# skhu101/SHERF

Measured on AMD Instinct MI355X. Metric: rendered rays/sec at 512x512x64 samples (ImportanceRenderer.forward), higher is better.
Workload: dtype f16 MFMA (fp16 operands rounded to nearest, one product, fp32 accumulate), fp32 elsewhere

## Files before the change

sherf_amd/csrc/mlp.hip:

```cpp
#include "common.h"

#include <algorithm>

namespace {

typedef __bf16 bf16x8 __attribute__((ext_vector_type(8)));
typedef __bf16 bf16x2 __attribute__((ext_vector_type(2)));
typedef _Float16 f16x8 __attribute__((ext_vector_type(8)));
typedef _Float16 f16x2 __attribute__((ext_vector_type(2)));
typedef float f32x16 __attribute__((ext_vector_type(16)));
typedef uint32_t u32x4 __attribute__((ext_vector_type(4)));

constexpr int N_CHUNKS = 49;
constexpr int N_STEPS = 43;
constexpr int NW = 4;
constexpr int NSLOT = 3;
constexpr int BIAS_LN = N_CHUNKS;

__host__ __device__ constexpr int step_units(int s) {
    return s < 4 ? 10 : s < 20 ? 8 : s < 26 ? ((s - 20) % 3 == 0 ? 10 : 8) : s < 42 ? 8 : 4;
}
__host__ __device__ constexpr int step_unit(int s, int u) {
    int c = -1, kb = 0;
    if (s == 0) { if (u < 2) { c = 0; kb = u; } else { c = 1 + (u - 2) / 2; kb = (u - 2) % 2; } }
// ... 294 lines not shown
        AFrag<PREC> nxt;
        const bool pre = i + 1 < NB || MORE;
        if (pre) nxt = load_units<PREC>(s + (u0 + 2 * (i + 1)) * UNIT);
        const BFrag<PREC>& b0 = b[PAIR ? i : 2 * i];
        const BFrag<PREC>& b1 = b[PAIR ? i : 2 * i + 1];
        if constexpr (PREC == 1) mfma_block<PREC>(acc0, acc1, cur.h0, cur.l0, cur.h1, cur.l1, b0.hi, b0.lo, b1.hi, b1.lo);
        else mfma_block<PREC>(acc0, acc1, cur.h0, cur.h0, cur.h1, cur.h1, b0.hi, b0.hi, b1.hi, b1.hi);
        if (pre) cur = nxt;
    }
}
template <int PREC, int NK, bool MORE = false>
__device__ __forceinline__ void mma_pair(const char* s, int u0, const BFrag<PREC>* b, f32x16& acc0, f32x16& acc1, AFrag<PREC>& cur) {
    mma_chains<PREC, NK, true, MORE>(s, u0, b, acc0, acc1, cur);
}
template <int PREC, int NK>
__device__ __forceinline__ void mma_splitk(const char* s, int u0, const BFrag<PREC>* b, f32x16& acc0, f32x16& acc1, AFrag<PREC>& cur) {
    static_assert(NK % 2 == 0, "even / odd K-block chains");
    mma_chains<PREC, NK / 2, false, false>(s, u0, b, acc0, acc1, cur);
}

#ifndef SHERF_MLP_PERMLANE
#define SHERF_MLP_PERMLANE 1
#endif
__device__ __forceinline__ float xhalf_sum(float v) {
#if SHERF_MLP_PERMLANE
    const uint32_t b = __builtin_bit_cast(uint32_t, v);
    const auto r = __builtin_amdgcn_permlane32_swap(b, b, false, false);
    return __builtin_bit_cast(float, (uint32_t)r[0]) + __builtin_bit_cast(float, (uint32_t)r[1]);
#else
    return v + __shfl_xor(v, 32);
#endif
}

template <int PREC, class C>
__device__ __forceinline__ void layer_norm(const C& cx, const f32x16& x, int ln_idx, BFrag<PREC>& k0, BFrag<PREC>& k1) {
    const f32x16 g = bias_tile(cx, BIAS_LN + 2 * ln_idx), bt = bias_tile(cx, BIAS_LN + 2 * ln_idx + 1);
    f32x16 y;
    if constexpr (PREC == 1) {
        float s = 0.f;
#pragma unroll
        for (int r = 0; r < 16; ++r) s += x[r];
        s = xhalf_sum(s);
        const float mean = s * (1.0f / 32.0f);
        float q = 0.f;
#pragma unroll
        for (int r = 0; r < 16; ++r) { float d = x[r] - mean; q += d * d; }
        q = xhalf_sum(q);
        const float inv = rsqrt_(q * (1.0f / 32.0f) + 1e-5f);
#pragma unroll
        for (int r = 0; r < 16; ++r) y[r] = (x[r] - mean) * inv * g[r] + bt[r];
    } else {
        float s = 0.f, q = 0.f;
#pragma unroll
        for (int r = 0; r < 16; ++r) { s += x[r]; q = __builtin_fmaf(x[r], x[r], q); }
        s = xhalf_sum(s); q = xhalf_sum(q);
        const float mean = s * (1.0f / 32.0f), ex2 = q * (1.0f / 32.0f);
        float var = fmaxf(__builtin_fmaf(-mean, mean, ex2), 0.0f);
        if (__ballot(ex2 > 257.0f * var) != 0) {
            float q2 = 0.f;
#pragma unroll
            for (int r = 0; r < 16; ++r) { const float d = x[r] - mean; q2 = __builtin_fmaf(d, d, q2); }
            var = xhalf_sum(q2) * (1.0f / 32.0f);
        }
        const float inv = rsqrt_(var + 1e-5f), off = -mean * inv;
#pragma unroll
        for (int r = 0; r < 16; ++r) y[r] = __builtin_fmaf(__builtin_fmaf(x[r], inv, off), g[r], bt[r]);
    }
    split_tile<PREC>(y, k0, k1);
}

__device__ __forceinline__ void sincos_exact_phase(float a, float* s, float* c) { sherf_sincos_exact_phase(a, s, c); }

template <int PREC, int NF, int NKB>
__device__ __forceinline__ void pe_frags(int h, float x, float y, float z, BFrag<PREC> (&out)[NKB]) {
    if constexpr ((SHERF_MLP_ABLATE & 512) != 0) {
#pragma unroll
        for (int kb = 0; kb < NKB; ++kb) out[kb] = make_frag<PREC>(x, y, z, 0.f, 0.f, 0.f, 0.f, 0.f);
        return;
    }
    float f[NKB * 16];
#pragma unroll
    for (int i = 0; i < NKB * 16; ++i) f[i] = 0.f;
    f[0] = x; f[1] = y; f[2] = z;
    const float v3[3] = {x, y, z};
#pragma unroll
    for (int q = 0; q < NF; ++q) {
#pragma unroll
        for (int a = 0; a < 3; ++a) {
            float s, c;
            sincos_exact_phase(v3[a] * (float)(1 << q), &s, &c);
            if (3 + 6 * q + a < NKB * 16) f[3 + 6 * q + a] = s;
            if (6 + 6 * q + a < NKB * 16) f[6 + 6 * q + a] = c;
        }
    }
#pragma unroll
    for (int kb = 0; kb < NKB; ++kb) {
        float v[8];
#pragma unroll
        for (int e = 0; e < 8; ++e) v[e] = h ? f[16 * kb + 8 + e] : f[16 * kb + e];
        out[kb] = make_frag<PREC>(v[0], v[1], v[2], v[3], v[4], v[5], v[6], v[7]);
    }
}

#ifndef SHERF_MLP_PK_RELU
#define SHERF_MLP_PK_RELU 1
#endif
__device__ __forceinline__ uint32_t relu2_f16(uint32_t p) {
    f16x2 v = __builtin_bit_cast(f16x2, p);
    v = __builtin_elementwise_max(v, f16x2{(_Float16)0.0f, (_Float16)0.0f});
    return __builtin_bit_cast(uint32_t, v);
}

template <int PREC, bool RELU>
__device__ __forceinline__ void finish_pair(f32x16& acc0, f32x16& acc1, BFrag<PREC>* out) {
    mfma_settle(acc0, acc1);
    if constexpr ((SHERF_MLP_ABLATE & 1024) != 0) {
#pragma unroll
        for (int f = 0; f < 4; ++f)
#pragma unroll
            for (int e = 0; e < 4; ++e) out[f].hi[e] = __builtin_bit_cast(uint32_t, f < 2 ? acc0[4 * f + e] : acc1[4 * (f - 2) + e]);
        __builtin_amdgcn_sched_barrier(0);
        return;
    }
    constexpr bool PK = RELU && PREC == 2 && SHERF_MLP_PK_RELU;
    if constexpr (RELU && !PK) {
// ... 23 lines not shown
template <int PREC, bool RING, bool PRE = false, bool PEM = false>
__device__ __forceinline__ void transformer_tile(Ctx<PREC>& cx, const float4* __restrict__ tokens, const float* __restrict__ extras, int64_t tile,
                                                 BFrag<PREC> (&z0b)[2], BFrag<PREC> (&z1b)[2], f32x16 (&tok)[3], const u32x4* __restrict__ pef = nullptr) {
    const int j = cx.lane & 31, h = cx.h;
    if (cx.notrans) {
        if constexpr (!PRE) load_tokens(tokens, tile, j, h, tok);
        split_tile<PREC>(tok[0], z0b[0], z0b[1]);
        split_tile<PREC>(tok[1], z1b[0], z1b[1]);
        if constexpr (RING) { advance(cx, 0); advance(cx, 1); }
        __builtin_amdgcn_sched_barrier(0);
        return;
    }
    {
        if constexpr (!PRE) load_tokens(tokens, tile, j, h, tok);
        const float* ex = extras + tile * 12 * 32 + j;
        if constexpr ((SHERF_MLP_ABLATE & 256) != 0) {
            split_tile<PREC>(tok[0] + tok[2], z0b[0], z0b[1]);
            split_tile<PREC>(tok[1] + tok[2], z1b[0], z1b[1]);
            if constexpr (RING) { advance(cx, 0); advance(cx, 1); }
            return;
        }

        const char* s = RING ? cx.slot(0) : cx.lds;
        {
            BFrag<PREC> b[1][2];
            if constexpr (PEM) { b[0][0].hi = pef[(tile * 7 + 5) * 64 + cx.lane]; b[0][1].hi = pef[(tile * 7 + 6) * 64 + cx.lane]; }
            else pe_frags<PREC, 5, 2>(h, ex[192], ex[224], ex[256], b[0]);
            f32x16 acc[1] = {bias_tile(cx, 0)};
            mma_cols<PREC, 2, 1>(s, 0, b, acc);
            tok[2] += acc[0];
        }
        BFrag<PREC> ln[3][2];
#pragma unroll
        for (int t = 0; t < 3; ++t) layer_norm<PREC>(cx, tok[t], 0, ln[t][0], ln[t][1]);
        float qa[2][16], qb[2][8];
        {
            BFrag<PREC> b2[2][2] = {{ln[0][0], ln[0][1]}, {ln[1][0], ln[1][1]}};
            f32x16 acc[2] = {bias_tile(cx, 1), bias_tile(cx, 1)};
            mma_cols<PREC, 2, 2>(s, 2, b2, acc);
#pragma unroll
            for (int i = 0; i < 2; ++i)
#pragma unroll
                for (int r = 0; r < 16; ++r) qa[i][r] = acc[i][r];
            f32x16 acc2[2] = {bias_tile(cx, 2), bias_tile(cx, 2)};
            mma_cols<PREC, 2, 2>(s, 4, b2, acc2);
#pragma unroll
            for (int i = 0; i < 2; ++i)
#pragma unroll
                for (int r = 0; r < 8; ++r) qb[i][r] = acc2[i][r];
        }
        float dot[2][3][3];
        float o[2][3][8];
        float v0[3][8];
#pragma unroll
        for (int t = 0; t < 3; ++t) {
            const BFrag<PREC> (&lt)[1][2] = reinterpret_cast<const BFrag<PREC> (&)[1][2]>(ln[t]);
            f32x16 acc[1] = {bias_tile(cx, 3)};
            mma_cols<PREC, 2, 1>(s, 6, lt, acc);
#pragma unroll
            for (int i = 0; i < 2; ++i) {
                float d0 = 0.f, d1 = 0.f;
#pragma unroll
                for (int r = 0; r < 8; ++r) { d0 += qa[i][r] * acc[0][r]; d1 += qa[i][8 + r] * acc[0][8 + r]; }
                dot[i][0][t] = d0; dot[i][1][t] = d1;
            }
        }
#pragma unroll
        for (int t = 0; t < 3; ++t) {
            const BFrag<PREC> (&lt)[1][2] = reinterpret_cast<const BFrag<PREC> (&)[1][2]>(ln[t]);
            f32x16 acc[1] = {bias_tile(cx, 4)};
            mma_cols<PREC, 2, 1>(s, 8, lt, acc);
#pragma unroll
            for (int i = 0; i < 2; ++i) {
                float d2 = 0.f;
#pragma unroll
                for (int r = 0; r < 8; ++r) d2 += qb[i][r] * acc[0][r];
                dot[i][2][t] = d2;
            }
#pragma unroll
            for (int r = 0; r < 8; ++r) v0[t][r] = acc[0][8 + r];
        }
        if constexpr (RING) advance(cx, 0);
#pragma unroll
        for (int i = 0; i < 2; ++i)
#pragma unroll
            for (int hd = 0; hd < 3; ++hd) {
                float d[3];
#pragma unroll
                for (int t = 0; t < 3; ++t) d[t] = xhalf_sum(dot[i][hd][t]) * 0.25f;
                float m = fmaxf(d[0], fmaxf(d[1], d[2]));
                float e0 = exp_(d[0] - m), e1 = exp_(d[1] - m), e2 = exp_(d[2] - m);
                float inv = rcp_(e0 + e1 + e2);
                dot[i][hd][0] = e0 * inv; dot[i][hd][1] = e1 * inv; dot[i][hd][2] = e2 * inv;
            }
#pragma unroll
        for (int i = 0; i < 2; ++i)
#pragma unroll
            for (int r = 0; r < 8; ++r) o[i][0][r] = dot[i][0][0] * v0[0][r] + dot[i][0][1] * v0[1][r] + dot[i][0][2] * v0[2][r];
        s = RING ? cx.slot(1) : cx.lds + step_pieces<PREC>(0) * 1024;
#pragma unroll
        for (int i = 0; i < 2; ++i)
#pragma unroll
            for (int r = 0; r < 8; ++r) { o[i][1][r] = 0.f; o[i][2][r] = 0.f; }
#pragma unroll
        for (int t = 0; t < 3; ++t) {
            const BFrag<PREC> (&lt)[1][2] = reinterpret_cast<const BFrag<PREC> (&)[1][2]>(ln[t]);
            f32x16 acc[1] = {bias_tile(cx, 5)};
            mma_cols<PREC, 2, 1>(s, 0, lt, acc);
#pragma unroll
            for (int i = 0; i < 2; ++i)
#pragma unroll
                for (int r = 0; r < 8; ++r) {
                    o[i][1][r] += dot[i][1][t] * acc[0][r];
                    o[i][2][r] += dot[i][2][t] * acc[0][8 + r];
                }
        }
        f32x16 y[2];
        {
            BFrag<PREC> ob[2][3];
#pragma unroll
            for (int i = 0; i < 2; ++i)
#pragma unroll
// ... 31 lines not shown
#pragma unroll
                for (int r = 0; r < 16; ++r) acc[i][r] = gelu_<PREC != 1>(acc[i][r]);
                split_tile<PREC>(acc[i], gb[i][0], gb[i][1]);
            }
            f32x16 acc2[2] = {bias_tile(cx, 8), bias_tile(cx, 8)};
            mma_cols<PREC, 2, 2>(s, 7, gb, acc2);
            if constexpr (RING) advance(cx, 1);
            f32x16 za = acc2[0] + y[0], zb = acc2[1] + y[1];
            split_tile<PREC>(za, z0b[0], z0b[1]);
            split_tile<PREC>(zb, z1b[0], z1b[1]);
        }
    }
    __builtin_amdgcn_sched_barrier(0);
}

template <int PREC>
__device__ __forceinline__ void decoder_tile(Ctx<PREC>& cx, const int32_t* __restrict__ counters, const BFrag<PREC> (&z0b)[2], const BFrag<PREC> (&z1b)[2],
                                             const float (&xc)[3], const float (&vc)[3], int64_t tile, bool live, int64_t nv, float4* __restrict__ out) {
    const int j = cx.lane & 31, h = cx.h;
    if constexpr (SHERF_MLP_DECODER_PRIO > 0) __builtin_amdgcn_s_setprio(SHERF_MLP_DECODER_PRIO);
    int step = 2;
    BFrag<PREC> ha[8], hb[8];
    AFrag<PREC> cur = load_units<PREC>(cx.slot(step));
#define SHERF_NEXT_STEP() do { step_wait(cx, step); cur = load_units<PREC>(cx.slot(step + 1)); dma_issue(cx, step + NSLOT); ++step; } while (0)
#define SHERF_LAYER128(C0, IN, OUT, RELU)                                                             \
    _Pragma("unroll") for (int P = 0; P < 2; ++P) {                                                   \
        f32x16 acc0 = bias_tile(cx, (C0) + 2 * P), acc1 = bias_tile(cx, (C0) + 2 * P + 1);            \
        mma_pair<PREC, 4>(cx.slot(step), 0, IN, acc0, acc1, cur);                                     \
        SHERF_NEXT_STEP();                                                                            \
        mma_pair<PREC, 4>(cx.slot(step), 0, IN + 4, acc0, acc1, cur);                                 \
        SHERF_NEXT_STEP();                                                                            \
        finish_pair<PREC, RELU>(acc0, acc1, OUT + 4 * P);                                             \
    }
    {
        BFrag<PREC> pe[3];
        pe_frags<PREC, 6, 3>(h, xc[0], xc[1], xc[2], pe);
#pragma unroll
        for (int P = 0; P < 2; ++P) {
            f32x16 acc0 = bias_tile(cx, 9 + 2 * P), acc1 = bias_tile(cx, 10 + 2 * P);
            const char* s = cx.slot(step);
            mma_pair<PREC, 3, true>(s, 0, pe, acc0, acc1, cur);
            mma_pair<PREC, 2>(s, 6, z0b, acc0, acc1, cur);
            SHERF_NEXT_STEP();
            finish_pair<PREC, true>(acc0, acc1, ha + 4 * P);
        }
    }
    SHERF_LAYER128(13, ha, hb, true)
    SHERF_LAYER128(17, hb, ha, true)
    SHERF_LAYER128(21, ha, hb, true)
    SHERF_LAYER128(25, hb, ha, true)
    {
        float x0 = xc[0], x1 = xc[1], x2 = xc[2];
        asm volatile("" : "+v"(x0), "+v"(x1), "+v"(x2));
        BFrag<PREC> pe[3];
        pe_frags<PREC, 6, 3>(h, x0, x1, x2, pe);
#pragma unroll
        for (int P = 0; P < 2; ++P) {
            f32x16 acc0 = bias_tile(cx, 29 + 2 * P), acc1 = bias_tile(cx, 30 + 2 * P);
            const char* s = cx.slot(step);
            mma_pair<PREC, 3, true>(s, 0, pe, acc0, acc1, cur);
            mma_pair<PREC, 2>(s, 6, z0b, acc0, acc1, cur);
            SHERF_NEXT_STEP();
            mma_pair<PREC, 4>(cx.slot(step), 0, ha, acc0, acc1, cur);
            SHERF_NEXT_STEP();
            mma_pair<PREC, 4>(cx.slot(step), 0, ha + 4, acc0, acc1, cur);
            SHERF_NEXT_STEP();
            finish_pair<PREC, true>(acc0, acc1, hb + 4 * P);
        }
    }
    SHERF_LAYER128(33, hb, ha, true)
    SHERF_LAYER128(37, ha, hb, true)
    SHERF_LAYER128(41, hb, ha, false)
    float sigma;
    {
        f32x16 acc0 = bias_tile(cx, 45), acc1 = {0.f, 0.f, 0.f, 0.f, 0.f, 0.f, 0.f, 0.f, 0.f, 0.f, 0.f, 0.f, 0.f, 0.f, 0.f, 0.f};
        mma_splitk<PREC, 8>(cx.slot(step), 0, hb, acc0, acc1, cur);
        SHERF_NEXT_STEP();
        mfma_settle(acc0, acc1);
        sigma = acc0[0] + acc1[0];
        __builtin_amdgcn_sched_barrier(0);
    }
    BFrag<PREC> gb[4];
    {
        BFrag<PREC> pv[2];
        pe_frags<PREC, 4, 2>(h, vc[0], vc[1], vc[2], pv);
        f32x16 acc0 = bias_tile(cx, 46), acc1 = bias_tile(cx, 47);
        mma_pair<PREC, 4>(cx.slot(step), 0, ha, acc0, acc1, cur);
        SHERF_NEXT_STEP();
// ... 53 lines not shown
        __builtin_amdgcn_sched_barrier(0);
        fill(f0 + i);
        __builtin_amdgcn_sched_barrier(0);
        if (pre) cur = nxt;
    }
}

template <int PREC, bool PEM = false>
__device__ __forceinline__ void decoder_tile_p(Ctx<PREC>& cx, const int32_t* __restrict__ counters, const BFrag<PREC> (&z0b)[2], const BFrag<PREC> (&z1b)[2],
                                               const float (&xc)[3], const float (&vc)[3], int64_t tile, bool live, int64_t nv, float4* __restrict__ out,
                                               const u32x4* __restrict__ pef = nullptr) {
    const int j = cx.lane & 31, h = cx.h;
    if constexpr (SHERF_MLP_DECODER_PRIO > 0) __builtin_amdgcn_s_setprio(SHERF_MLP_DECODER_PRIO);
    int step = 2;
    BFrag<PREC> ha[8], hb[8];
    if constexpr ((SHERF_MLP_ABLATE & 2048) != 0) {
#pragma unroll
        for (int i = 0; i < 8; ++i) { ha[i] = z0b[i & 1]; hb[i] = z1b[i & 1]; }
    }
    f32x16 X0, X1, Y0, Y1;
    AFrag<PREC> cur = load_units<PREC>(cx.slot(step));
    const f32x16 zero = {0.f, 0.f, 0.f, 0.f, 0.f, 0.f, 0.f, 0.f, 0.f, 0.f, 0.f, 0.f, 0.f, 0.f, 0.f, 0.f};
    auto none = [](int) {};
#define SHERF_NEXT_STEP() do { step_wait(cx, step); cur = load_units<PREC>(cx.slot(step + 1)); dma_issue(cx, step + NSLOT); ++step; } while (0)
#define SHERF_LAYER128_P(C0, IN, OUT, RELU, PREV_RELU, NX0, NX1)                                                                              \
    mma_chains_f<PREC, 4, true, false>(cx.slot(step), 0, IN, X0, X1, cur, 0, [&](int i) { epi_piece<PREC, PREV_RELU>(Y0, Y1, IN + 4, i); }); \
    SHERF_NEXT_STEP();                                                                                                                         \
    mma_chains_f<PREC, 4, true, false>(cx.slot(step), 0, IN + 4, X0, X1, cur, 0, [&](int i) { if (i == 0) { Y0 = bias_tile(cx, (C0) + 2); Y1 = bias_tile(cx, (C0) + 3); } }); \
    SHERF_NEXT_STEP();                                                                                                                         \
    mma_chains_f<PREC, 4, true, false>(cx.slot(step), 0, IN, Y0, Y1, cur, 0, [&](int i) { epi_piece<PREC, RELU>(X0, X1, OUT, i); });           \
    SHERF_NEXT_STEP();                                                                                                                         \
    mma_chains_f<PREC, 4, true, false>(cx.slot(step), 0, IN + 4, Y0, Y1, cur, 0, [&](int i) { if (i == 0) { X0 = bias_tile(cx, NX0); X1 = (NX1) < 0 ? zero : bias_tile(cx, (NX1) < 0 ? 0 : (NX1)); } }); \
    SHERF_NEXT_STEP();
    {
        BFrag<PREC> pe[3];
        if constexpr (PEM) {
#pragma unroll
            for (int kb = 0; kb < 3; ++kb) pe[kb].hi = pef[(tile * 7 + kb) * 64];
        } else pe_frags<PREC, 6, 3>(h, xc[0], xc[1], xc[2], pe);
        X0 = bias_tile(cx, 9); X1 = bias_tile(cx, 10);
        const char* s = cx.slot(step);
        mma_chains_f<PREC, 3, true, true>(s, 0, pe, X0, X1, cur, 0, [&](int i) { if (i == 0) { Y0 = bias_tile(cx, 11); Y1 = bias_tile(cx, 12); } });
        mma_chains_f<PREC, 2, true, false>(s, 6, z0b, X0, X1, cur, 3, none);
        SHERF_NEXT_STEP();
        s = cx.slot(step);
        auto carry = [&](int i) { if (i < 4) epi_piece<PREC, true>(X0, X1, ha, i); else { X0 = bias_tile(cx, 13); X1 = bias_tile(cx, 14); } };
        mma_chains_f<PREC, 3, true, true>(s, 0, pe, Y0, Y1, cur, 0, carry);
        mma_chains_f<PREC, 2, true, false>(s, 6, z0b, Y0, Y1, cur, 3, carry);
        SHERF_NEXT_STEP();
    }
    SHERF_LAYER128_P(13, ha, hb, true, true, 17, 18)
    SHERF_LAYER128_P(17, hb, ha, true, true, 21, 22)
    SHERF_LAYER128_P(21, ha, hb, true, true, 25, 26)
    SHERF_LAYER128_P(25, hb, ha, true, true, 29, 30)
    {
        float x0 = xc[0], x1 = xc[1], x2 = xc[2];
        asm volatile("" : "+v"(x0), "+v"(x1), "+v"(x2));
        BFrag<PREC> pe[3];
        if constexpr (PEM) {
            const u32x4* pp = pef;
            asm volatile("" : "+v"(pp));
#pragma unroll
            for (int kb = 0; kb < 3; ++kb) pe[kb].hi = pp[(tile * 7 + kb) * 64];
        } else pe_frags<PREC, 6, 3>(h, x0, x1, x2, pe);
        const char* s = cx.slot(step);
        auto carry0 = [&](int i) { if (i < 4) epi_piece<PREC, true>(Y0, Y1, ha + 4, i); };
        mma_chains_f<PREC, 3, true, true>(s, 0, pe, X0, X1, cur, 0, carry0);
        mma_chains_f<PREC, 2, true, false>(s, 6, z0b, X0, X1, cur, 3, carry0);
        SHERF_NEXT_STEP();
        mma_chains_f<PREC, 4, true, false>(cx.slot(step), 0, ha, X0, X1, cur, 0, [&](int i) { if (i == 0) { Y0 = bias_tile(cx, 31); Y1 = bias_tile(cx, 32); } });
        SHERF_NEXT_STEP();
        mma_chains_f<PREC, 4, true, false>(cx.slot(step), 0, ha + 4, X0, X1, cur, 0, none);
        SHERF_NEXT_STEP();
        s = cx.slot(step);
        auto carry1 = [&](int i) { if (i < 4) epi_piece<PREC, true>(X0, X1, hb, i); };
        mma_chains_f<PREC, 3, true, true>(s, 0, pe, Y0, Y1, cur, 0, carry1);
        mma_chains_f<PREC, 2, true, false>(s, 6, z0b, Y0, Y1, cur, 3, carry1);
        SHERF_NEXT_STEP();
        mma_chains_f<PREC, 4, true, false>(cx.slot(step), 0, ha, Y0, Y1, cur, 0, [&](int i) { if (i == 0) { X0 = bias_tile(cx, 33); X1 = bias_tile(cx, 34); } });
        SHERF_NEXT_STEP();
        mma_chains_f<PREC, 4, true, false>(cx.slot(step), 0, ha + 4, Y0, Y1, cur, 0, none);
        SHERF_NEXT_STEP();
    }
    SHERF_LAYER128_P(33, hb, ha, true, true, 37, 38)
    SHERF_LAYER128_P(37, ha, hb, true, true, 41, 42)
    SHERF_LAYER128_P(41, hb, ha, false, true, 45, -1)
    float sigma;
    BFrag<PREC> gb[4];
    {
        mma_chains_f<PREC, 4, false, false>(cx.slot(step), 0, hb, X0, X1, cur, 0, [&](int i) {
            epi_piece<PREC, false>(Y0, Y1, ha + 4, i);
            if (i == 3) { Y0 = bias_tile(cx, 46); Y1 = bias_tile(cx, 47); }
        });
        SHERF_NEXT_STEP();
        BFrag<PREC> pv[2];
        if constexpr (PEM) { pv[0].hi = pef[(tile * 7 + 3) * 64]; pv[1].hi = pef[(tile * 7 + 4) * 64]; }
        else pe_frags<PREC, 4, 2>(h, vc[0], vc[1], vc[2], pv);
// ... 467 lines not shown
            z1b[kb].hi = zp[(4 + 2 * kb) * 64]; z1b[kb].lo = zp[(4 + 2 * kb + 1) * 64];
        } else {
            z0b[kb].hi = zp[kb * 64]; z1b[kb].hi = zp[(2 + kb) * 64];
        }
    }
    float xc[3], vc[3];
    const float* ex = extras + tile * 12 * 32 + (cx.lane & 31);
    xc[0] = ex[0]; xc[1] = ex[32]; xc[2] = ex[64]; vc[0] = ex[96]; vc[1] = ex[128]; vc[2] = ex[160];
    decoder_tile<PREC>(cx, counters, z0b, z1b, xc, vc, tile, live, nv, out);
    SHERF_TRACE_FLUSH(cx);
}

}

#if SHERF_MLP_TRACE
extern "C" int sherf_mlp_set_trace(void* buf, int every) {
    SHERF_HIP_CHECK(hipMemcpyToSymbol(HIP_SYMBOL(g_mlp_trace), &buf, sizeof(buf)));
    SHERF_HIP_CHECK(hipMemcpyToSymbol(HIP_SYMBOL(g_mlp_trace_every), &every, sizeof(every)));
    return SHERF_OK;
}
#endif

extern "C" int sherf_mlp_stream_layout(int prec, int32_t* n_steps, int32_t* step_pieces_host, int32_t* units, int32_t max_steps) {
    SHERF_CHECK_ARG(prec >= 0 && prec <= 2 && n_steps && step_pieces_host && units && max_steps >= N_STEPS);
    *n_steps = N_STEPS;
    for (int s = 0; s < N_STEPS; ++s) {
        step_pieces_host[s] = prec == 1 ? step_pieces<1>(s) : step_pieces<0>(s);
        for (int u = 0; u < 10; ++u) units[s * 10 + u] = u < step_units(s) ? step_unit(s, u) : -1;
    }
    return SHERF_OK;
}

namespace {
__global__ void __launch_bounds__(256) mlp_pack_stream_kernel(const float* __restrict__ flat, const int32_t* __restrict__ src, int64_t n16, int prec,
                                                              uint16_t* __restrict__ out, const int32_t* __restrict__ bias_src, int n_bias,
                                                              float* __restrict__ bias_out, int32_t* __restrict__ flag) {
    const int64_t i = (int64_t)blockIdx.x * 256 + threadIdx.x;
    int bad = 0;
    if (i < n16) {
        const int32_t sidx = src[i];
        uint16_t bits = 0;
        if (sidx >= 0) {
            const float v = flat[sidx >> 1];
            if (!(fabsf(v) <= 3.0e38f)) bad |= 1;
            if (prec == 0) {
                const uint32_t b = __float_as_uint(v);
                bits = (uint16_t)((b + 0x7FFFu + ((b >> 16) & 1u)) >> 16);
            } else {
                if (fabsf(v) > 65504.0f) bad |= 2;
                const _Float16 hi = (_Float16)v;
                const _Float16 pc = (sidx & 1) ? (_Float16)(v - (float)hi) : hi;
                bits = __builtin_bit_cast(uint16_t, pc);
            }
        }
        out[i] = bits;
    }
    if (i < n_bias) {
        const int32_t b = bias_src[i];
        const float v = b >= 0 ? flat[b] : 0.f;
        if (!(fabsf(v) <= 3.0e38f)) bad |= 1;
        bias_out[i] = v;
    }
    if (bad) atomicOr(reinterpret_cast<unsigned*>(flag), (unsigned)bad);
}
}

extern "C" int sherf_mlp_pack_stream(const float* flat, const int32_t* src, int64_t n_slots, int prec, void* stream_out,
                                     const int32_t* bias_src, int n_bias, float* bias_out, int32_t* flag, sherf_stream_t stream) {
    SHERF_CHECK_ARG(flat && src && stream_out && bias_src && bias_out && flag && n_slots > 0 && n_bias > 0 && n_bias <= n_slots);
    SHERF_CHECK_ARG(prec >= 0 && prec <= 2);
    SHERF_HIP_CHECK(hipMemsetAsync(flag, 0, sizeof(int32_t), as_stream(stream)));
    hipLaunchKernelGGL(mlp_pack_stream_kernel, dim3((unsigned)((n_slots + 255) / 256)), dim3(256), 0, as_stream(stream), flat, src, n_slots, prec,
                       reinterpret_cast<uint16_t*>(stream_out), bias_src, n_bias, bias_out, flag);
    SHERF_LAUNCH_CHECK();
}

extern "C" int sherf_nerf_mlp_part(const int32_t* counters, const float* tokens, const float* extras, const void* wstream,
                                   const float* wbias, int prec, int64_t capacity, float* out, int part, int nparts, sherf_stream_t stream) {
    SHERF_CHECK_ARG(counters && tokens && extras && wstream && wbias && out);
    const int notrans = (prec & SHERF_MLP_NO_TRANSFORMER) ? 1 : 0;
    prec &= ~SHERF_MLP_NO_TRANSFORMER;
    SHERF_CHECK_ARG(prec >= 0 && prec <= 2 && capacity > 0 && nparts >= 0 && nparts < 256 && (nparts <= 1 || (part >= 0 && part < nparts)));
    const int64_t tiles = nparts > 1 ? ((capacity + 255) / 256 + nparts - 1) / nparts * 8 + 8 : (capacity + 31) / 32;
    const dim3 grid((unsigned)((tiles + NW - 1) / NW)), block(NW * 64);
    if (prec == 1)
        hipLaunchKernelGGL((nerf_mlp_kernel<1>), grid, block, 0, as_stream(stream), counters, reinterpret_cast<const float4*>(tokens), extras,
                           reinterpret_cast<const char*>(wstream), wbias, capacity, reinterpret_cast<float4*>(out), part, nparts, notrans);
    else if (prec == 2)
        hipLaunchKernelGGL((nerf_mlp_kernel<2>), grid, block, 0, as_stream(stream), counters, reinterpret_cast<const float4*>(tokens), extras,
                           reinterpret_cast<const char*>(wstream), wbias, capacity, reinterpret_cast<float4*>(out), part, nparts, notrans);
    else
        hipLaunchKernelGGL((nerf_mlp_kernel<0>), grid, block, 0, as_stream(stream), counters, reinterpret_cast<const float4*>(tokens), extras,
// ... 100 lines not shown
```

sherf_amd/mlp_pack.py:

```python
import numpy as np

N_CHUNKS = 49


def _bf16_bits(x):
    b = np.ascontiguousarray(x, dtype=np.float32).view(np.uint32)
    return ((b + 0x7FFF + ((b >> 16) & 1)) >> 16).astype(np.uint16)


def _bf16_val(x):
    return (_bf16_bits(x).astype(np.uint32) << 16).view(np.float32)


def dlay_feature(kb, h, e):
    return 16 * kb + (e & 3) + 8 * (e >> 2) + 4 * h


def nat_feature(kb, h, e):
    return 16 * kb + 8 * h + e


def chunk_specs(sd, r='renderer.', d='decoder.', dtype=np.float32):
    g = lambda n: np.asarray(sd[n], dtype=dtype)
    ident = list(range(32))
    specs = []

    def add(W, rows, segs, bias=None):
        specs.append(dict(W=W, rows=list(rows) + [-1] * (32 - len(rows)), segs=segs, bias=bias))

    Wr = g(r + 'conv1d_reprojection.weight')[:, :, 0]
    add(Wr[:, 32:64], ident, [('nat', 0, 2, 32)])
    t = r + 'transformer.layers.0.'
    Wqkv = g(t + '0.fn.fn.to_qkv.weight')
    for rows in (range(0, 32), range(32, 48), range(48, 80), range(80, 112), range(112, 144)):
        add(Wqkv, rows, [('dlay', 0, 2, 32)])
    add(g(t + '0.fn.fn.to_out.0.weight'), ident, [('dlay', 0, 3, 48)], g(t + '0.fn.fn.to_out.0.bias'))
    add(g(t + '1.fn.fn.net.0.weight'), ident, [('dlay', 0, 2, 32)], g(t + '1.fn.fn.net.0.bias'))
    add(g(t + '1.fn.fn.net.3.weight'), ident, [('dlay', 0, 2, 32)], g(t + '1.fn.fn.net.3.bias'))
    x0 = [('nat', 0, 3, 39), ('dlay', 39, 2, 32)]
    for L in range(8):
        W, b = g(f'{d}pts_linears.{L}.weight'), g(f'{d}pts_linears.{L}.bias')
        segs = x0 if L == 0 else (x0 + [('dlay', 71, 8, 128)] if L == 5 else [('dlay', 0, 8, 128)])
        for T in range(4):
            add(W, range(32 * T, 32 * T + 32), segs, b)
    Wf, bf = g(d + 'feature_linear.weight'), g(d + 'feature_linear.bias')
    for T in range(4):
        add(Wf, range(32 * T, 32 * T + 32), [('dlay', 0, 8, 128)], bf)
    add(g(d + 'alpha_linear.weight'), [0], [('dlay', 0, 8, 128)], g(d + 'alpha_linear.bias'))
    Wv, bv = g(d + 'views_linear.weight'), g(d + 'views_linear.bias')
    for T in range(2):
        add(Wv, range(32 * T, 32 * T + 32), [('dlay', 0, 8, 128), ('nat', 128, 2, 27), ('dlay', 155, 2, 32)], bv)
    add(g(d + 'rgb_linear.weight'), [0, 1, 2], [('dlay', 0, 4, 64)], g(d + 'rgb_linear.bias'))
    assert len(specs) == N_CHUNKS
    return specs


def chunk_nkb(spec):
    return sum(s[2] for s in spec['segs'])


def chunk_image(spec, fill=0):
    W = spec['W']
    nkb = chunk_nkb(spec)
    img = np.full((nkb, 64, 8), fill, W.dtype)
    kb0 = 0
    for kind, base, n, real in spec['segs']:
        for kb in range(n):
            for l in range(64):
                i, h = l & 31, l >> 5
                row = spec['rows'][i]
                if row < 0:
                    continue
                for e in range(8):
                    f = dlay_feature(kb, h, e) if kind == 'dlay' else nat_feature(kb, h, e)
                    if f < real:
                        img[kb0 + kb, l, e] = W[row, base + f]
        kb0 += n
    return img


def bias_table(vec, rows, fill=0):
    out = np.full((2, 16), fill, np.float32 if vec is None else np.asarray(vec).dtype)
    if vec is None:
        return out
    for h in range(2):
        for rr in range(16):
            row = rows[(rr & 3) + 8 * (rr >> 2) + 4 * h]
            if row >= 0:
                out[h, rr] = vec[row]
    return out


N_STEPS = 43
PRECISIONS = {'bf16': 0, 'f16x3': 1, 'f16': 2}
N_PIECE = {0: 1, 1: 2, 2: 1}


def step_units(s):
    return 10 if s < 4 else 8 if s < 20 else (10 if (s - 20) % 3 == 0 else 8) if s < 26 else 8 if s < 42 else 4


def step_unit(s, u):
    if s == 0:
        return (0, u) if u < 2 else (1 + (u - 2) // 2, (u - 2) % 2)
    if s == 1:
        return (5, u) if u < 2 else (6, u - 2) if u < 5 else (7, u - 5) if u < 7 else (8, u - 7) if u < 9 else None
    if s < 4:
        return (9 + 2 * (s - 2) + (u & 1), u // 2)
    if s < 20:
        q = s - 4
        return (13 + 4 * (q // 4) + 2 * ((q % 4) // 2) + (u & 1), 4 * (q % 2) + u // 2)
    if s < 26:
        q = s - 20
        return (29 + 2 * (q // 3) + (u & 1), (0, 5, 9)[q % 3] + u // 2)
    if s < 34:
        q = s - 26
        return (33 + 4 * (q // 4) + 2 * ((q % 4) // 2) + (u & 1), 4 * (q % 2) + u // 2)
    if s < 38:
        q = s - 34
        return (41 + 2 * (q // 2) + (u & 1), 4 * (q % 2) + u // 2)
    if s == 38:
        return (45, u)
# ... 13 lines not shown
F16_MAX = 65504.0


def check_f16_range(sd, r='renderer.', d='decoder.', prec=1):
    if prec == 0:
        return
    bound = 64.0
    for name, v in sd.items():
        if not (name.startswith(d) or name.startswith(r + 'transformer') or name.startswith(r + 'conv1d_reprojection')):
            continue
        a = np.asarray(v, dtype=np.float32)
        if not np.isfinite(a).all():
            raise ValueError(f'{name}: non-finite values; the MLP weight stream cannot be packed')
        if a.size and float(np.abs(a).max()) > F16_MAX:
            raise ValueError(f'{name}: |w| up to {float(np.abs(a).max()):.3g} exceeds the fp16 range of mlp_precision f16x3 / f16; use bf16')
    for lname in [f'{d}pts_linears.{i}' for i in range(8)] + [d + 'feature_linear', d + 'views_linear']:
        W = np.abs(np.asarray(sd[lname + '.weight'], np.float64)).sum(1).max()
        bound = bound * W + np.abs(np.asarray(sd[lname + '.bias'], np.float64)).max()
    if bound > 1e30:
        raise ValueError(f'decoder weight norms allow activations up to ~{bound:.1e}: outside the fp16 range of mlp_precision f16x3 / f16; use bf16')


def raise_for_flags(flag, bound, prec):
    if flag & 1:
        raise ValueError('non-finite values in the transformer / decoder weights; the MLP weight stream cannot be packed')
    if prec != 0 and (flag & 2):
        raise ValueError('a transformer / decoder weight exceeds the fp16 range of mlp_precision f16x3 / f16; use bf16')
    if prec != 0 and bound > 1e30:
        raise ValueError(f'decoder weight norms allow activations up to ~{bound:.1e}: outside the fp16 range of mlp_precision f16x3 / f16; use bf16')


def pack(sd, r='renderer.', d='decoder.', prec=1):
    assert prec in (0, 1, 2)
    check_f16_range(sd, r, d, prec)
    specs = chunk_specs(sd, r, d)
    frag, bias, nkbs = [], [], []
    for sp in specs:
        img = chunk_image(sp)
        if prec == 1:
            hi = _f16_bits(img)
            lo = _f16_bits(img - hi.view(np.float16).astype(np.float32))
        elif prec == 2:
            hi, lo = _f16_bits(img), None
        else:
            hi, lo = _bf16_bits(img), None
        frag.append((hi, lo))
        bias.append(bias_table(sp['bias'], sp['rows']))
        nkbs.append(img.shape[0])
    parts, used = [], set()
    for s_ in range(N_STEPS):
        n = 0
        for u in range(step_units(s_)):
            cu = step_unit(s_, u)
            if cu is None:
                parts.append(bytes(1024 * N_PIECE[prec]))
            else:
                c, kb = cu
                assert kb < nkbs[c] and cu not in used, (s_, u, cu)
                used.add(cu)
                parts.append(frag[c][0][kb].tobytes())
                if prec == 1:
                    parts.append(frag[c][1][kb].tobytes())
            n += N_PIECE[prec]
        parts.append(bytes(1024 * (step_pieces(s_, prec) - n)))
    assert len(used) == sum(nkbs), 'every (chunk, K-block) unit must be streamed exactly once'
    t = r + 'transformer.layers.0.'
    for n in ('0.fn.norm.weight', '0.fn.norm.bias', '1.fn.norm.weight', '1.fn.norm.bias'):
        bias.append(bias_table(np.asarray(sd[t + n], np.float32), list(range(32))))
    stream = np.frombuffer(b''.join(parts), dtype=np.uint8).copy()
    return stream, np.stack(bias).reshape(-1).astype(np.float32), nkbs


_NORM_NAMES = ('0.fn.norm.weight', '0.fn.norm.bias', '1.fn.norm.weight', '1.fn.norm.bias')


def packed_names(r='renderer.', d='decoder.'):
    t = r + 'transformer.layers.0.'
    names = [r + 'conv1d_reprojection.weight', t + '0.fn.fn.to_qkv.weight', t + '0.fn.fn.to_out.0.weight', t + '0.fn.fn.to_out.0.bias',
             t + '1.fn.fn.net.0.weight', t + '1.fn.fn.net.0.bias', t + '1.fn.fn.net.3.weight', t + '1.fn.fn.net.3.bias']
    for L in range(8):
        names += [f'{d}pts_linears.{L}.weight', f'{d}pts_linears.{L}.bias']
    for n in ('feature_linear', 'alpha_linear', 'views_linear', 'rgb_linear'):
        names += [d + n + '.weight', d + n + '.bias']
    return names + [t + n for n in _NORM_NAMES]


_index_cache = {}


def stream_index(shapes, r='renderer.', d='decoder.', prec=1):
    names = packed_names(r, d)
    key = (prec, r, d, tuple(tuple(shapes[n]) for n in names))
    if key in _index_cache:
        return _index_cache[key]
    sd, off = {}, 0
    for n in names:
        k = int(np.prod(shapes[n]))
        sd[n] = np.arange(off, off + k, dtype=np.int64).reshape(tuple(shapes[n]))
        off += k
    specs = chunk_specs(sd, r, d, dtype=np.int64)
    imgs = [chunk_image(sp, fill=-1) for sp in specs]
    npc = N_PIECE[prec]
    pad = np.full(512, -1, np.int64)
    parts = []
    for s_ in range(N_STEPS):
        n = 0
        for u in range(step_units(s_)):
            cu = step_unit(s_, u)
            for q in range(npc):
                if cu is None:
                    parts.append(pad)
                else:
                    e = imgs[cu[0]][cu[1]].reshape(-1)
                    parts.append(np.where(e >= 0, 2 * e + q, -1))
            n += npc
        parts += [pad] * (step_pieces(s_, prec) - n)
    src = np.concatenate(parts).astype(np.int32)
    bias = [bias_table(sp['bias'], sp['rows'], fill=-1).astype(np.int64) if sp['bias'] is not None else np.full((2, 16), -1, np.int64)
            for sp in specs]
    t = r + 'transformer.layers.0.'
    bias += [bias_table(sd[t + n], list(range(32)), fill=-1) for n in _NORM_NAMES]
    out = (src, np.stack(bias).reshape(-1).astype(np.int32), off)
    _index_cache[key] = out
    return out


def pack_from_index(flat, src, bias_src, prec):
    flat = np.asarray(flat, np.float32)
    v = np.where(src >= 0, flat[np.maximum(src, 0) >> 1], np.float32(0)).astype(np.float32)
    if prec == 0:
        bits = _bf16_bits(v)
    else:
        hi = v.astype(np.float16)
        bits = np.where((src & 1) == 1, (v - hi.astype(np.float32)).astype(np.float16).view(np.uint16), hi.view(np.uint16))
        bits = np.where(src >= 0, bits, 0).astype(np.uint16)
    wb = np.where(bias_src >= 0, flat[np.maximum(bias_src, 0)], np.float32(0)).astype(np.float32)
    return bits.view(np.uint8), wb
```

Measured before the change: 166.1 million.

## Fold LayerNorm affine and attention scale into weights, share PE sincos across half-waves

```diff
diff --git a/sherf_amd/csrc/mlp.hip b/sherf_amd/csrc/mlp.hip
--- a/sherf_amd/csrc/mlp.hip
+++ b/sherf_amd/csrc/mlp.hip
@@ -350,11 +350,16 @@
 #endif
 }
 
+#ifndef SHERF_MLP_FOLD
+#define SHERF_MLP_FOLD 1
+#endif
+template <int PREC> constexpr bool FOLD_LN = SHERF_MLP_FOLD && PREC != 1;
+template <int PREC> constexpr bool FOLD_SCALE = SHERF_MLP_FOLD && PREC == 2;
 template <int PREC, class C>
 __device__ __forceinline__ void layer_norm(const C& cx, const f32x16& x, int ln_idx, BFrag<PREC>& k0, BFrag<PREC>& k1) {
-    const f32x16 g = bias_tile(cx, BIAS_LN + 2 * ln_idx), bt = bias_tile(cx, BIAS_LN + 2 * ln_idx + 1);
     f32x16 y;
     if constexpr (PREC == 1) {
+        const f32x16 g = bias_tile(cx, BIAS_LN + 2 * ln_idx), bt = bias_tile(cx, BIAS_LN + 2 * ln_idx + 1);
         float s = 0.f;
 #pragma unroll
         for (int r = 0; r < 16; ++r) s += x[r];
@@ -382,13 +387,24 @@
         }
         const float inv = rsqrt_(var + 1e-5f), off = -mean * inv;
 #pragma unroll
-        for (int r = 0; r < 16; ++r) y[r] = __builtin_fmaf(__builtin_fmaf(x[r], inv, off), g[r], bt[r]);
+        for (int r = 0; r < 16; ++r) y[r] = __builtin_fmaf(x[r], inv, off);
+        if constexpr (!FOLD_LN<PREC>) {
+            const f32x16 g = bias_tile(cx, BIAS_LN + 2 * ln_idx), bt = bias_tile(cx, BIAS_LN + 2 * ln_idx + 1);
+#pragma unroll
+            for (int r = 0; r < 16; ++r) y[r] = __builtin_fmaf(y[r], g[r], bt[r]);
+        }
     }
     split_tile<PREC>(y, k0, k1);
 }
 
 __device__ __forceinline__ void sincos_exact_phase(float a, float* s, float* c) { sherf_sincos_exact_phase(a, s, c); }
 
+#ifndef SHERF_MLP_PE_SPLIT
+#define SHERF_MLP_PE_SPLIT SHERF_MLP_PERMLANE
+#endif
+#ifndef SHERF_MLP_PE_ONCE
+#define SHERF_MLP_PE_ONCE 1
+#endif
 template <int PREC, int NF, int NKB>
 __device__ __forceinline__ void pe_frags(int h, float x, float y, float z, BFrag<PREC> (&out)[NKB]) {
     if constexpr ((SHERF_MLP_ABLATE & 512) != 0) {
@@ -400,15 +416,39 @@
 #pragma unroll
     for (int i = 0; i < NKB * 16; ++i) f[i] = 0.f;
     f[0] = x; f[1] = y; f[2] = z;
-    const float v3[3] = {x, y, z};
-#pragma unroll
-    for (int q = 0; q < NF; ++q) {
-#pragma unroll
-        for (int a = 0; a < 3; ++a) {
-            float s, c;
-            sincos_exact_phase(v3[a] * (float)(1 << q), &s, &c);
-            if (3 + 6 * q + a < NKB * 16) f[3 + 6 * q + a] = s;
-            if (6 + 6 * q + a < NKB * 16) f[6 + 6 * q + a] = c;
+    constexpr bool SPLIT = SHERF_MLP_PE_SPLIT && PREC != 1;
+    if constexpr (SPLIT) {
+#if SHERF_MLP_PE_SPLIT
+        constexpr int NH = (NF + 1) / 2;
+        const float up = h ? (float)(1 << NH) : 1.0f;
+        const float w3[3] = {x * up, y * up, z * up};
+#pragma unroll
+        for (int q = 0; q < NH; ++q) {
+#pragma unroll
+            for (int a = 0; a < 3; ++a) {
+                float s, c;
+                sincos_exact_phase(w3[a] * (float)(1 << q), &s, &c);
+                const uint32_t sb = __builtin_bit_cast(uint32_t, s), cb = __builtin_bit_cast(uint32_t, c);
+                const auto rs = __builtin_amdgcn_permlane32_swap(sb, sb, false, false);
+                const auto rc = __builtin_amdgcn_permlane32_swap(cb, cb, false, false);
+                if (3 + 6 * q + a < NKB * 16) f[3 + 6 * q + a] = __builtin_bit_cast(float, (uint32_t)rs[0]);
+                if (6 + 6 * q + a < NKB * 16) f[6 + 6 * q + a] = __builtin_bit_cast(float, (uint32_t)rc[0]);
+                if (q + NH < NF && 3 + 6 * (q + NH) + a < NKB * 16) f[3 + 6 * (q + NH) + a] = __builtin_bit_cast(float, (uint32_t)rs[1]);
+                if (q + NH < NF && 6 + 6 * (q + NH) + a < NKB * 16) f[6 + 6 * (q + NH) + a] = __builtin_bit_cast(float, (uint32_t)rc[1]);
+            }
+        }
+#endif
+    } else {
+        const float v3[3] = {x, y, z};
+#pragma unroll
+        for (int q = 0; q < NF; ++q) {
+#pragma unroll
+            for (int a = 0; a < 3; ++a) {
+                float s, c;
+                sincos_exact_phase(v3[a] * (float)(1 << q), &s, &c);
+                if (3 + 6 * q + a < NKB * 16) f[3 + 6 * q + a] = s;
+                if (6 + 6 * q + a < NKB * 16) f[6 + 6 * q + a] = c;
+            }
         }
     }
 #pragma unroll
@@ -498,7 +538,10 @@
         }
         BFrag<PREC> ln[3][2];
 #pragma unroll
-        for (int t = 0; t < 3; ++t) layer_norm<PREC>(cx, tok[t], 0, ln[t][0], ln[t][1]);
+        for (int t = 0; t < 3; ++t) {
+            layer_norm<PREC>(cx, tok[t], 0, ln[t][0], ln[t][1]);
+            if constexpr (FOLD_LN<PREC>) __builtin_amdgcn_sched_barrier(0);
+        }
         float qa[2][16], qb[2][8];
         {
             BFrag<PREC> b2[2][2] = {{ln[0][0], ln[0][1]}, {ln[1][0], ln[1][1]}};
@@ -553,7 +596,7 @@
             for (int hd = 0; hd < 3; ++hd) {
                 float d[3];
 #pragma unroll
-                for (int t = 0; t < 3; ++t) d[t] = xhalf_sum(dot[i][hd][t]) * 0.25f;
+                for (int t = 0; t < 3; ++t) d[t] = FOLD_SCALE<PREC> ? xhalf_sum(dot[i][hd][t]) : xhalf_sum(dot[i][hd][t]) * 0.25f;
                 float m = fmaxf(d[0], fmaxf(d[1], d[2]));
                 float e0 = exp_(d[0] - m), e1 = exp_(d[1] - m), e2 = exp_(d[2] - m);
                 float inv = rcp_(e0 + e1 + e2);
@@ -651,8 +694,10 @@
         SHERF_NEXT_STEP();                                                                            \
         finish_pair<PREC, RELU>(acc0, acc1, OUT + 4 * P);                                             \
     }
-    {
-        BFrag<PREC> pe[3];
+    constexpr bool PE_ONCE = SHERF_MLP_PE_ONCE && PREC != 1;
+    BFrag<PREC> pe6[3];
+    {
+        BFrag<PREC> (&pe)[3] = pe6;
         pe_frags<PREC, 6, 3>(h, xc[0], xc[1], xc[2], pe);
 #pragma unroll
         for (int P = 0; P < 2; ++P) {
@@ -669,10 +714,13 @@
     SHERF_LAYER128(21, ha, hb, true)
     SHERF_LAYER128(25, hb, ha, true)
     {
-        float x0 = xc[0], x1 = xc[1], x2 = xc[2];
-        asm volatile("" : "+v"(x0), "+v"(x1), "+v"(x2));
-        BFrag<PREC> pe[3];
-        pe_frags<PREC, 6, 3>(h, x0, x1, x2, pe);
+        BFrag<PREC> pe5[3];
+        if constexpr (!PE_ONCE) {
+            float x0 = xc[0], x1 = xc[1], x2 = xc[2];
+            asm volatile("" : "+v"(x0), "+v"(x1), "+v"(x2));
+            pe_frags<PREC, 6, 3>(h, x0, x1, x2, pe5);
+        }
+        const BFrag<PREC> (&pe)[3] = PE_ONCE ? pe6 : pe5;
 #pragma unroll
         for (int P = 0; P < 2; ++P) {
             f32x16 acc0 = bias_tile(cx, 29 + 2 * P), acc1 = bias_tile(cx, 30 + 2 * P);
@@ -792,8 +840,10 @@
     SHERF_NEXT_STEP();                                                                                                                         \
     mma_chains_f<PREC, 4, true, false>(cx.slot(step), 0, IN + 4, Y0, Y1, cur, 0, [&](int i) { if (i == 0) { X0 = bias_tile(cx, NX0); X1 = (NX1) < 0 ? zero : bias_tile(cx, (NX1) < 0 ? 0 : (NX1)); } }); \
     SHERF_NEXT_STEP();
-    {
-        BFrag<PREC> pe[3];
+    constexpr bool PE_ONCE = SHERF_MLP_PE_ONCE && !PEM;
+    BFrag<PREC> pe6[3];
+    {
+        BFrag<PREC> (&pe)[3] = pe6;
         if constexpr (PEM) {
 #pragma unroll
             for (int kb = 0; kb < 3; ++kb) pe[kb].hi = pef[(tile * 7 + kb) * 64];
@@ -814,15 +864,18 @@
     SHERF_LAYER128_P(21, ha, hb, true, true, 25, 26)
     SHERF_LAYER128_P(25, hb, ha, true, true, 29, 30)
     {
-        float x0 = xc[0], x1 = xc[1], x2 = xc[2];
-        asm volatile("" : "+v"(x0), "+v"(x1), "+v"(x2));
-        BFrag<PREC> pe[3];
+        BFrag<PREC> pe5[3];
         if constexpr (PEM) {
             const u32x4* pp = pef;
             asm volatile("" : "+v"(pp));
 #pragma unroll
-            for (int kb = 0; kb < 3; ++kb) pe[kb].hi = pp[(tile * 7 + kb) * 64];
-        } else pe_frags<PREC, 6, 3>(h, x0, x1, x2, pe);
+            for (int kb = 0; kb < 3; ++kb) pe5[kb].hi = pp[(tile * 7 + kb) * 64];
+        } else if constexpr (!PE_ONCE) {
+            float x0 = xc[0], x1 = xc[1], x2 = xc[2];
+            asm volatile("" : "+v"(x0), "+v"(x1), "+v"(x2));
+            pe_frags<PREC, 6, 3>(h, x0, x1, x2, pe5);
+        }
+        const BFrag<PREC> (&pe)[3] = PE_ONCE ? pe6 : pe5;
         const char* s = cx.slot(step);
         auto carry0 = [&](int i) { if (i < 4) epi_piece<PREC, true>(Y0, Y1, ha + 4, i); };
         mma_chains_f<PREC, 3, true, true>(s, 0, pe, X0, X1, cur, 0, carry0);
@@ -1356,16 +1409,21 @@
 }
 
 namespace {
+constexpr int32_t PACK_ELEM = (1 << 20) - 1, PACK_ONE = 1 << 29, PACK_DOT = 1 << 30;
 __global__ void __launch_bounds__(256) mlp_pack_stream_kernel(const float* __restrict__ flat, const int32_t* __restrict__ src, int64_t n16, int prec,
                                                               uint16_t* __restrict__ out, const int32_t* __restrict__ bias_src, int n_bias,
                                                               float* __restrict__ bias_out, int32_t* __restrict__ flag) {
     const int64_t i = (int64_t)blockIdx.x * 256 + threadIdx.x;
+    const int ln0 = n_bias > N_CHUNKS * 32 && bias_src[N_CHUNKS * 32] >= 0 ? bias_src[N_CHUNKS * 32] & PACK_ELEM : 0;
     int bad = 0;
     if (i < n16) {
         const int32_t sidx = src[i];
         uint16_t bits = 0;
         if (sidx >= 0) {
-            const float v = flat[sidx >> 1];
+            float v = flat[(sidx >> 1) & PACK_ELEM];
+            const int gain = (sidx >> 21) & 127;
+            if (gain) v = v * flat[ln0 + (gain - 1) / 32 * 64 + (gain - 1) % 32];
+            if ((sidx >> 28) & 1) v = v * 0.25f;
             if (!(fabsf(v) <= 3.0e38f)) bad |= 1;
             if (prec == 0) {
                 const uint32_t b = __float_as_uint(v);
@@ -1381,7 +1439,15 @@
     }
     if (i < n_bias) {
         const int32_t b = bias_src[i];
-        const float v = b >= 0 ? flat[b] : 0.f;
+        float v = 0.f;
+        if (b >= 0 && (b & PACK_ONE)) v = 1.0f;
+        else if (b >= 0 && (b & PACK_DOT)) {
+            const int e = b & PACK_ELEM, row = (b >> 20) & 31, bt = ln0 + 64 * ((b >> 26) & 1) + 32;
+            double acc = (b >> 25) & 1 ? (double)flat[e + (32 - row) * 32 + row] : 0.0;
+            for (int c = 0; c < 32; ++c) acc += (double)flat[e + c] * (double)flat[bt + c];
+            v = (float)acc;
+            if ((b >> 27) & 1) v = v * 0.25f;
+        } else if (b >= 0) v = flat[b];
         if (!(fabsf(v) <= 3.0e38f)) bad |= 1;
         bias_out[i] = v;
     }
diff --git a/sherf_amd/mlp_pack.py b/sherf_amd/mlp_pack.py
--- a/sherf_amd/mlp_pack.py
+++ b/sherf_amd/mlp_pack.py
@@ -32,8 +32,9 @@
     add(Wr[:, 32:64], ident, [('nat', 0, 2, 32)])
     t = r + 'transformer.layers.0.'
     Wqkv = g(t + '0.fn.fn.to_qkv.weight')
+    bqkv = g(t + QKV_BIAS) if t + QKV_BIAS in sd else None
     for rows in (range(0, 32), range(32, 48), range(48, 80), range(80, 112), range(112, 144)):
-        add(Wqkv, rows, [('dlay', 0, 2, 32)])
+        add(Wqkv, rows, [('dlay', 0, 2, 32)], bqkv)
     add(g(t + '0.fn.fn.to_out.0.weight'), ident, [('dlay', 0, 3, 48)], g(t + '0.fn.fn.to_out.0.bias'))
     add(g(t + '1.fn.fn.net.0.weight'), ident, [('dlay', 0, 2, 32)], g(t + '1.fn.fn.net.0.bias'))
     add(g(t + '1.fn.fn.net.3.weight'), ident, [('dlay', 0, 2, 32)], g(t + '1.fn.fn.net.3.bias'))
@@ -88,6 +89,70 @@
             row = rows[(rr & 3) + 8 * (rr >> 2) + 4 * h]
             if row >= 0:
                 out[h, rr] = vec[row]
+    return out
+
+
+QKV_BIAS = '0.fn.fn.to_qkv.bias'
+Q_ROWS = 48
+FOLD_LN = {0: True, 1: False, 2: True}
+FOLD_SCALE = {0: False, 1: False, 2: True}
+
+
+def _fold_dot(W, bt, b0=None):
+    acc = np.zeros(W.shape[0], np.float64) if b0 is None else np.asarray(b0, np.float64).copy()
+    for c in range(W.shape[1]):
+        acc += W[:, c].astype(np.float64) * np.float64(bt[c])
+    return acc.astype(np.float32)
+
+
+def fold_state(sd, r='renderer.', prec=1):
+    if not FOLD_LN[prec] and not FOLD_SCALE[prec]:
+        return sd
+    t = r + 'transformer.layers.0.'
+    out = dict(sd)
+    f = lambda n: np.asarray(sd[t + n], np.float32)
+    Wq, W1, b1 = f('0.fn.fn.to_qkv.weight'), f('1.fn.fn.net.0.weight'), f('1.fn.fn.net.0.bias')
+    bq = np.zeros(Wq.shape[0], np.float32)
+    if FOLD_LN[prec]:
+        bq = _fold_dot(Wq, f('0.fn.norm.bias'))
+        b1 = _fold_dot(W1, f('1.fn.norm.bias'), b1)
+        Wq, W1 = Wq * f('0.fn.norm.weight')[None, :], W1 * f('1.fn.norm.weight')[None, :]
+        for n, v in (('0.fn.norm.weight', 1), ('0.fn.norm.bias', 0), ('1.fn.norm.weight', 1), ('1.fn.norm.bias', 0)):
+            out[t + n] = np.full(32, v, np.float32)
+    if FOLD_SCALE[prec]:
+        Wq, bq = Wq.copy(), bq.copy()
+        Wq[:Q_ROWS] *= np.float32(0.25); bq[:Q_ROWS] *= np.float32(0.25)
+    out[t + '0.fn.fn.to_qkv.weight'], out[t + QKV_BIAS] = Wq.astype(np.float32), bq.astype(np.float32)
+    out[t + '1.fn.fn.net.0.weight'], out[t + '1.fn.fn.net.0.bias'] = W1.astype(np.float32), b1.astype(np.float32)
+    return out
+
+
+ELEM_BITS = 20
+BIAS_ONE, BIAS_DOT = 1 << 29, 1 << 30
+
+
+def fold_index(sd, r='renderer.', prec=1):
+    if not FOLD_LN[prec] and not FOLD_SCALE[prec]:
+        return sd
+    t = r + 'transformer.layers.0.'
+    out = dict(sd)
+    Wq, W1, b1 = sd[t + '0.fn.fn.to_qkv.weight'], sd[t + '1.fn.fn.net.0.weight'], sd[t + '1.fn.fn.net.0.bias']
+    assert Wq.shape[1] == 32 and W1.shape == (32, 32) and max(int(v.max()) for v in sd.values()) < (1 << ELEM_BITS)
+    ln0 = int(sd[t + _NORM_NAMES[0]][0])
+    assert all(int(sd[t + n][0]) == ln0 + 32 * i for i, n in enumerate(_NORM_NAMES)), 'the four norm vectors must be contiguous'
+    scale = (np.arange(Wq.shape[0]) < Q_ROWS).astype(np.int64) if FOLD_SCALE[prec] else np.zeros(Wq.shape[0], np.int64)
+    col = np.arange(32, dtype=np.int64)
+    if FOLD_LN[prec]:
+        rows = np.arange(32, dtype=np.int64)
+        assert np.array_equal(b1, W1[:, 0] + (32 - rows) * 32 + rows), 'net.0.bias must follow net.0.weight in the flat vector'
+        out[t + QKV_BIAS] = BIAS_DOT | Wq[:, 0] | (scale << 27)
+        out[t + '1.fn.fn.net.0.bias'] = BIAS_DOT | W1[:, 0] | (rows << ELEM_BITS) | (1 << 25) | (1 << 26)
+        out[t + '0.fn.fn.to_qkv.weight'] = Wq | ((1 + col) << ELEM_BITS)[None, :] | (scale << 27)[:, None]
+        out[t + '1.fn.fn.net.0.weight'] = W1 | ((33 + col) << ELEM_BITS)[None, :]
+        for i, n in enumerate(_NORM_NAMES):
+            out[t + n] = (BIAS_ONE | sd[t + n]) if i % 2 == 0 else np.full(32, -1, np.int64)
+    else:
+        out[t + '0.fn.fn.to_qkv.weight'] = Wq | (scale << 27)[:, None]
     return out
 
 
@@ -167,6 +232,7 @@
 
 def pack(sd, r='renderer.', d='decoder.', prec=1):
     assert prec in (0, 1, 2)
+    sd = fold_state(sd, r, prec)
     check_f16_range(sd, r, d, prec)
     specs = chunk_specs(sd, r, d)
     frag, bias, nkbs = [], [], []
@@ -233,6 +299,7 @@
         k = int(np.prod(shapes[n]))
         sd[n] = np.arange(off, off + k, dtype=np.int64).reshape(tuple(shapes[n]))
         off += k
+    sd = fold_index(sd, r, prec)
     specs = chunk_specs(sd, r, d, dtype=np.int64)
     imgs = [chunk_image(sp, fill=-1) for sp in specs]
     npc = N_PIECE[prec]
@@ -262,12 +329,32 @@
 
 def pack_from_index(flat, src, bias_src, prec):
     flat = np.asarray(flat, np.float32)
-    v = np.where(src >= 0, flat[np.maximum(src, 0) >> 1], np.float32(0)).astype(np.float32)
+    src, bias_src = np.asarray(src, np.int64), np.asarray(bias_src, np.int64)
+    emask = (1 << ELEM_BITS) - 1
+    ln0 = int(bias_src[N_CHUNKS * 32]) & emask
+    ok, G = src >= 0, (np.maximum(src, 0) >> (ELEM_BITS + 1)) & 127
+    v = flat[(np.maximum(src, 0) >> 1) & emask]
+    v = np.where(G > 0, v * flat[np.minimum(ln0 + (G - 1) // 32 * 64 + (G - 1) % 32, flat.size - 1)], v).astype(np.float32)
+    v = np.where((np.maximum(src, 0) >> 28) & 1 == 1, v * np.float32(0.25), v)
+    v = np.where(ok, v, np.float32(0)).astype(np.float32)
     if prec == 0:
         bits = _bf16_bits(v)
     else:
         hi = v.astype(np.float16)
         bits = np.where((src & 1) == 1, (v - hi.astype(np.float32)).astype(np.float16).view(np.uint16), hi.view(np.uint16))
-        bits = np.where(src >= 0, bits, 0).astype(np.uint16)
-    wb = np.where(bias_src >= 0, flat[np.maximum(bias_src, 0)], np.float32(0)).astype(np.float32)
+        bits = np.where(ok, bits, 0).astype(np.uint16)
+    wb = np.zeros(bias_src.size, np.float32)
+    for i, b in enumerate(bias_src.tolist()):
+        if b < 0:
+            continue
+        if b & BIAS_ONE:
+            wb[i] = 1.0
+        elif b & BIAS_DOT:
+            e, row, ln = b & emask, (b >> ELEM_BITS) & 31, (b >> 26) & 1
+            acc = np.float64(flat[e + (32 - row) * 32 + row]) if (b >> 25) & 1 else np.float64(0)
+            for c in range(32):
+                acc += np.float64(flat[e + c]) * np.float64(flat[ln0 + 64 * ln + 32 + c])
+            wb[i] = np.float32(acc) * (np.float32(0.25) if (b >> 27) & 1 else np.float32(1))
+        else:
+            wb[i] = flat[b]
     return bits.view(np.uint8), wb
```

Measured after the change: 163.7 million. 0.985x the previous value.
